# wx-ys/pynbody-extras

Hardware: AMD Instinct MI355X
Metric: particle-pairs/sec (direct-sum gravity, force+potential) (higher is better)
Workload: dtype f64; 1 GPU; 1000000-particle Plummer sphere, direct-sum force+potential (Newtonian), 1000000 targets/GPU x 1000000 sources; n_particles=1000000, seed=1002, parallelism=targets sharded x1, device=gfx950 device (gfx950:sramecc+:xnack-, 256 CUs)

## Files before the change

### pynbody-extras_amd/csrc/direct.hip

```cpp
#include <cstdlib>
#include <cstring>

#include "pbx_common.h"

namespace pbx {

static constexpr double kR2Tiny = 2.2250738585072014e-308;
static constexpr int kBlock = 256;

__device__ __forceinline__ double rsqrt_nr(double x) {
  double y = __builtin_amdgcn_rsq(x);
  double e = __builtin_fma(-x * y, y, 1.0);
  return __builtin_fma(0.5 * y, e, y);
}

__device__ __forceinline__ double w2_inner(double u) {
  double u2 = u * u;
  if (u < 0.5) {
    double u4 = u2 * u2;
    double u5 = u4 * u;
    return (16.0 / 3.0) * u2 - (48.0 / 5.0) * u4 + (32.0 / 5.0) * u5 - 14.0 / 5.0;
  }
  double inv_u = 1.0 / u;
  double u3 = u2 * u;
  double u4 = u2 * u2;
  double u5 = u4 * u;
  return (1.0 / 15.0) * inv_u + (32.0 / 3.0) * u2 - 16.0 * u3 + (48.0 / 5.0) * u4 -
         (32.0 / 15.0) * u5 - 16.0 / 5.0;
}

__device__ __forceinline__ double w2p_inner(double u) {
  double u2 = u * u;
  double u3 = u2 * u;
  double u4 = u2 * u2;
  if (u < 0.5) return (32.0 / 3.0) * u - (192.0 / 5.0) * u3 + 32.0 * u4;
  return -(1.0 / 15.0) * (1.0 / u2) + (64.0 / 3.0) * u - 48.0 * u2 + (192.0 / 5.0) * u3 -
         (32.0 / 3.0) * u4;
}

template <int KERN, int WANT>
__device__ __forceinline__ void pair(double dx, double dy, double dz, double m, double h,
                                     double &ph, double &ax, double &ay, double &az) {
  double s2 = __builtin_fma(dx, dx, __builtin_fma(dy, dy, __builtin_fma(dz, dz, kR2Tiny)));
  const double s = (KERN == 0) ? __builtin_fma(h, h, s2) : s2;
  const double y0 = __builtin_amdgcn_rsq(s);
  const double w = y0 * __builtin_fma(-s, y0 * y0, 3.0);
  double mw = m * w;
  double g8 = mw * (w * w);
  if (KERN == 1) {
    double r = s2 * (0.5 * w);
    if (!(h <= 0.0) && !(r >= h)) {
      double hinv = 1.0 / h;
      double u = r * hinv;
      mw = -2.0 * m * (w2_inner(u) * hinv);
      g8 = 8.0 * m * (w2p_inner(u) * (hinv * hinv) / r);
    }
  }
  if (WANT & PBX_WANT_POT) ph += mw;
  if (WANT & PBX_WANT_ACC) {
    ax = __builtin_fma(g8, dx, ax);
    ay = __builtin_fma(g8, dy, ay);
    az = __builtin_fma(g8, dz, az);
  }
}

template <int KERN, int WANT, bool CHECK, int T>
__device__ __forceinline__ void sweep(const double4 *__restrict__ src,
                                      const double *__restrict__ src_h, bool has_h,
                                      int64_t j0, int64_t j1, const double (&xi)[T],
                                      const double (&yi)[T], const double (&zi)[T],
                                      const double (&hi)[T], const int64_t (&me)[T],
                                      double (&ph)[T], double (&ax)[T], double (&ay)[T],
                                      double (&az)[T]) {
#pragma unroll 4
  for (int64_t j = j0; j < j1; ++j) {
    const double4 s = src[j];
    double hj = 0.0;
    if (KERN >= 0) hj = has_h ? src_h[j] : 0.0;
#pragma unroll
    for (int k = 0; k < T; ++k) {
      double dx = s.x - xi[k];
      double dy = s.y - yi[k];
      double dz = s.z - zi[k];
      double m = s.w;
      double h = 0.0;
      if (KERN >= 0) h = __builtin_fmax(hi[k], hj);
      if (CHECK) {
        bool self = (j == me[k]);
        m = self ? 0.0 : m;
        dx = self ? 1.0 : dx;
        if (KERN >= 0) h = self ? 0.0 : h;
      }
      pair<KERN, WANT>(dx, dy, dz, m, h, ph[k], ax[k], ay[k], az[k]);
    }
  }
}

template <int KERN, int WANT, bool SELF, int T>
__global__ void __launch_bounds__(kBlock)
    direct_kernel(const double4 *__restrict__ src, const double *__restrict__ src_h,
                  int has_h, int64_t n_src, int64_t chunk, const double *__restrict__ tgt,
                  const double *__restrict__ tgt_h, int64_t n_tgt, int64_t self_offset,
                  double *__restrict__ pot_out, double *__restrict__ acc_out,
                  int64_t out_split_stride) {
  const int64_t tbase = (int64_t)blockIdx.x * (kBlock * T);
  const int64_t js = (int64_t)blockIdx.y * chunk;
  const int64_t je = (js + chunk < n_src) ? js + chunk : n_src;

  double xi[T], yi[T], zi[T], hi[T], ph[T], ax[T], ay[T], az[T];
  int64_t me[T];
#pragma unroll
  for (int k = 0; k < T; ++k) {
    int64_t t = tbase + k * kBlock + threadIdx.x;
    int64_t tc = t < n_tgt ? t : n_tgt - 1;
    xi[k] = tgt[3 * tc + 0];
    yi[k] = tgt[3 * tc + 1];
    zi[k] = tgt[3 * tc + 2];
    hi[k] = (SELF && KERN >= 0 && has_h) ? tgt_h[tc] : 0.0;
    me[k] = SELF ? self_offset + t : -1;
    ph[k] = ax[k] = ay[k] = az[k] = 0.0;
  }

  const bool hh = has_h != 0;
  if (SELF) {
    int64_t d0 = self_offset + tbase;
    int64_t d1 = d0 + kBlock * T;
    d0 = d0 < js ? js : (d0 > je ? je : d0);
    d1 = d1 < js ? js : (d1 > je ? je : d1);
    sweep<KERN, WANT, false, T>(src, src_h, hh, js, d0, xi, yi, zi, hi, me, ph, ax, ay, az);
    sweep<KERN, WANT, true, T>(src, src_h, hh, d0, d1, xi, yi, zi, hi, me, ph, ax, ay, az);
    sweep<KERN, WANT, false, T>(src, src_h, hh, d1, je, xi, yi, zi, hi, me, ph, ax, ay, az);
  } else {
    sweep<KERN, WANT, false, T>(src, src_h, hh, js, je, xi, yi, zi, hi, me, ph, ax, ay, az);
  }

  const int64_t soff = (int64_t)blockIdx.y * out_split_stride;
#pragma unroll
  for (int k = 0; k < T; ++k) {
    int64_t t = tbase + k * kBlock + threadIdx.x;
    if (t < n_tgt) {
      if (WANT & PBX_WANT_POT) pot_out[soff + t] = -0.5 * ph[k];
      if (WANT & PBX_WANT_ACC) {
        double *a = acc_out + 3 * (soff + t);
        a[0] = 0.125 * ax[k];
        a[1] = 0.125 * ay[k];
        a[2] = 0.125 * az[k];
      }
    }
  }
}

template <int WANT>
__global__ void __launch_bounds__(kBlock)
    reduce_splits(const double *__restrict__ pot_part, const double *__restrict__ acc_part,
                  int nsplit, int64_t n_tgt, double *__restrict__ pot,
                  double *__restrict__ acc) {
  int64_t t = (int64_t)blockIdx.x * kBlock + threadIdx.x;
  if (t >= n_tgt) return;
  if (WANT & PBX_WANT_POT) {
    double s = 0.0;
    for (int k = 0; k < nsplit; ++k) s += pot_part[(int64_t)k * n_tgt + t];
    pot[t] = s;
  }
  if (WANT & PBX_WANT_ACC) {
    double sx = 0.0, sy = 0.0, sz = 0.0;
    for (int k = 0; k < nsplit; ++k) {
      const double *a = acc_part + 3 * ((int64_t)k * n_tgt + t);
      sx += a[0];
      sy += a[1];
      sz += a[2];
    }
    acc[3 * t + 0] = sx;
    acc[3 * t + 1] = sy;
    acc[3 * t + 2] = sz;
  }
}

__global__ void __launch_bounds__(kBlock)
    pack_sources_kernel(const double *__restrict__ pos, const double *__restrict__ mass,
                        int64_t n, double4 *__restrict__ rec) {
  int64_t i = (int64_t)blockIdx.x * kBlock + threadIdx.x;
  if (i >= n) return;
  rec[i] = make_double4(pos[3 * i + 0], pos[3 * i + 1], pos[3 * i + 2],
                        mass ? mass[i] : 1.0);
}

constexpr int kTargetsPerLane = 4;

template <int KERN, int WANT, bool SELF>
static void launch_variant(hipStream_t st, dim3 grid, const double4 *src, const double *src_h,
                           int has_h, int64_t n_src, int64_t chunk, const double *tgt,
                           const double *tgt_h, int64_t n_tgt, int64_t self_offset,
                           double *pot, double *acc, int64_t stride) {
  hipLaunchKernelGGL((direct_kernel<KERN, WANT, SELF, kTargetsPerLane>), grid, dim3(kBlock), 0,
                     st, src, src_h, has_h, n_src, chunk, tgt, tgt_h, n_tgt, self_offset, pot, acc,
                     stride);
}

template <int KERN, int WANT>
static void launch_self(bool self, hipStream_t st, dim3 grid, const double4 *src,
                        const double *src_h, int has_h, int64_t n_src, int64_t chunk,
                        const double *tgt, const double *tgt_h, int64_t n_tgt,
                        int64_t self_offset, double *pot, double *acc, int64_t stride) {
  if (self)
    launch_variant<KERN, WANT, true>(st, grid, src, src_h, has_h, n_src, chunk, tgt, tgt_h,
                                     n_tgt, self_offset, pot, acc, stride);
  else
    launch_variant<KERN, WANT, false>(st, grid, src, src_h, has_h, n_src, chunk, tgt, tgt_h,
                                      n_tgt, self_offset, pot, acc, stride);
}

template <int KERN>
static void launch_want(int want, bool self, hipStream_t st, dim3 grid, const double4 *src,
                        const double *src_h, int has_h, int64_t n_src, int64_t chunk,
                        const double *tgt, const double *tgt_h, int64_t n_tgt,
                        int64_t self_offset, double *pot, double *acc, int64_t stride) {
  switch (want) {
    case 1:
      launch_self<KERN, 1>(self, st, grid, src, src_h, has_h, n_src, chunk, tgt, tgt_h, n_tgt,
                           self_offset, pot, acc, stride);
      break;
    case 2:
      launch_self<KERN, 2>(self, st, grid, src, src_h, has_h, n_src, chunk, tgt, tgt_h, n_tgt,
                           self_offset, pot, acc, stride);
      break;
    default:
      launch_self<KERN, 3>(self, st, grid, src, src_h, has_h, n_src, chunk, tgt, tgt_h, n_tgt,
                           self_offset, pot, acc, stride);
      break;
  }
}

int64_t sym_padded(int64_t n);
int64_t sym_unit_count(int64_t n);
void sym_accumulate(Device &d, double4 *rec, int64_t n, int64_t u0, int64_t u1, int want,
                    double *acc4, DevBuf &unit_buf);
void sym_finish(Device &d, const double *acc4, int64_t lo, int64_t hi, int want, double *pot,
                double *acc);

static constexpr int64_t kSymMinN = 8192;

void direct_device(Device &d, const double *src, const double *src_h, int64_t n_src,
                   const double *tgt, const double *tgt_h, int64_t n_tgt, int64_t self_offset,
                   int kernel, int want, double *pot, double *acc) {
  if (n_tgt <= 0) return;
  hipStream_t st = d.stream;
  if (kernel == PBX_KERNEL_NONE && self_offset == 0 && n_tgt == n_src && n_src >= kSymMinN) {
    const int64_t npad = sym_padded(n_src);
    double4 *rec = (double4 *)d.slot(kSlotSymRec).ensure(sizeof(double4) * npad);
    double *acc4 = (double *)d.slot(kSlotSymAcc).ensure(sizeof(double) * 4 * npad);
    PBX_HIP(hipMemcpyAsync(rec, src, sizeof(double4) * n_src, hipMemcpyDeviceToDevice, st));
    PBX_HIP(hipMemsetAsync(acc4, 0, sizeof(double) * 4 * npad, st));
    sym_accumulate(d, rec, n_src, 0, sym_unit_count(n_src), want, acc4, d.slot(kSlotSymUnits));
    sym_finish(d, acc4, 0, n_src, want, pot, acc);
    return;
  }
  if (n_src <= 0) {
    if (want & PBX_WANT_POT) PBX_HIP(hipMemsetAsync(pot, 0, sizeof(double) * n_tgt, st));
    if (want & PBX_WANT_ACC) PBX_HIP(hipMemsetAsync(acc, 0, sizeof(double) * 3 * n_tgt, st));
    return;
  }
  const int64_t per_block = (int64_t)kBlock * kTargetsPerLane;
  const int64_t bx = (n_tgt + per_block - 1) / per_block;
  int64_t nsplit = (2048 + bx - 1) / bx;
  int64_t max_split = (n_src + 4095) / 4096;
  if (nsplit > max_split) nsplit = max_split;
  if (nsplit > 64) nsplit = 64;
  if (nsplit < 1) nsplit = 1;
  const int64_t chunk = (n_src + nsplit - 1) / nsplit;
  nsplit = (n_src + chunk - 1) / chunk;
  if (bx > 0x7fffffff) fail(PBX_ERR_VALUE, "too many targets (%lld)", (long long)n_tgt);
  dim3 grid((unsigned)bx, (unsigned)nsplit);
  const bool self = self_offset >= 0;
  const int has_h = src_h != nullptr;

  double *pot_k = pot, *acc_k = acc;
  int64_t stride = 0;
  if (nsplit > 1) {
    size_t per = 0;
    if (want & PBX_WANT_POT) per += 1;
    if (want & PBX_WANT_ACC) per += 3;
    double *part = (double *)d.slot(kSlotPart).ensure(sizeof(double) * per * nsplit * n_tgt);
    pot_k = (want & PBX_WANT_POT) ? part : nullptr;
    acc_k = (want & PBX_WANT_ACC) ? part + ((want & PBX_WANT_POT) ? nsplit * n_tgt : 0)
                                  : nullptr;
    stride = n_tgt;
  }
  const double4 *src4 = (const double4 *)src;
  switch (kernel) {
    case PBX_KERNEL_NONE:
      launch_want<-1>(want, self, st, grid, src4, src_h, has_h, n_src, chunk, tgt, tgt_h,
                      n_tgt, self_offset, pot_k, acc_k, stride);
      break;
    case PBX_KERNEL_PLUMMER:
      launch_want<0>(want, self, st, grid, src4, src_h, has_h, n_src, chunk, tgt, tgt_h,
                     n_tgt, self_offset, pot_k, acc_k, stride);
      break;
    case PBX_KERNEL_SPLINE:
      launch_want<1>(want, self, st, grid, src4, src_h, has_h, n_src, chunk, tgt, tgt_h,
                     n_tgt, self_offset, pot_k, acc_k, stride);
      break;
    default:
      fail(PBX_ERR_VALUE, "kernel must be 0 (Plummer) or 1 (CubicSplineW2)");
  }
  PBX_HIP(hipGetLastError());
  if (nsplit > 1) {
    dim3 rg(ceil_div(n_tgt, kBlock));
    switch (want) {
      case 1:
        hipLaunchKernelGGL(reduce_splits<1>, rg, dim3(kBlock), 0, st, pot_k, acc_k,
                           (int)nsplit, n_tgt, pot, acc);
        break;
      case 2:
        hipLaunchKernelGGL(reduce_splits<2>, rg, dim3(kBlock), 0, st, pot_k, acc_k,
                           (int)nsplit, n_tgt, pot, acc);
        break;
      default:
        hipLaunchKernelGGL(reduce_splits<3>, rg, dim3(kBlock), 0, st, pot_k, acc_k,
                           (int)nsplit, n_tgt, pot, acc);
        break;
    }
    PBX_HIP(hipGetLastError());
  }
}

void pack_sources_device(Device &d, const double *pos, const double *mass, int64_t n,
                         double *rec) {
  if (n <= 0) return;
  hipLaunchKernelGGL(pack_sources_kernel, dim3(ceil_div(n, kBlock)), dim3(kBlock), 0, d.stream,
                     pos, mass, n, (double4 *)rec);
  PBX_HIP(hipGetLastError());
}

static void check_kernel(int kernel, const double *soft) {
  if (kernel != PBX_KERNEL_NONE && kernel != PBX_KERNEL_PLUMMER && kernel != PBX_KERNEL_SPLINE)
    fail(PBX_ERR_VALUE, "kernel must be 0 (Plummer) or 1 (CubicSplineW2)");
  if (kernel == PBX_KERNEL_NONE && soft != nullptr)
    fail(PBX_ERR_VALUE,
         "softenings require an explicit kernel; pass kernel=0/1 (or omit softenings)");
}

static void direct_host(const double *h_pos, int64_t n, const double *h_tgt, int64_t m,
                        const double *h_mass, const double *h_soft, int kernel, int want,
                        double *h_out) {
  if (n < 0 || m < 0) fail(PBX_ERR_VALUE, "negative particle count");
  check_kernel(kernel, h_soft);
  const bool self = (h_tgt == nullptr);
  const int64_t n_tgt = self ? n : m;
  if (n_tgt == 0) return;
  Device &d = current_device();
  std::lock_guard<std::mutex> lk(d.mu);
  hipStream_t st = d.stream;
  size_t out_elems = (want == PBX_WANT_POT ? 1 : 3) * (size_t)n_tgt;
  if (n == 0) {
    std::memset(h_out, 0, sizeof(double) * out_elems);
    return;
  }
  ScopedTimer total("pbx.direct.total");
  double *d_pos = (double *)d.slot(kSlotPos).ensure(sizeof(double) * 3 * n);
  double *d_mass = h_mass ? (double *)d.slot(kSlotMass).ensure(sizeof(double) * n) : nullptr;
  double *d_src = (double *)d.slot(kSlotSrc).ensure(sizeof(double) * 4 * n);
  const bool use_h = h_soft != nullptr && kernel != PBX_KERNEL_NONE;
  double *d_src_h = use_h ? (double *)d.slot(kSlotSrcH).ensure(sizeof(double) * n) : nullptr;
  double *d_tgt = self ? d_pos : (double *)d.slot(kSlotTgt).ensure(sizeof(double) * 3 * m);
  double *d_out = (double *)d.slot(want == PBX_WANT_POT ? kSlotPot : kSlotAcc)
                      .ensure(sizeof(double) * out_elems);
  {
    ScopedTimer t("pbx.direct.h2d");
    PBX_HIP(hipMemcpyAsync(d_pos, h_pos, sizeof(double) * 3 * n, hipMemcpyHostToDevice, st));
    if (h_mass)
      PBX_HIP(hipMemcpyAsync(d_mass, h_mass, sizeof(double) * n, hipMemcpyHostToDevice, st));
    if (use_h)
      PBX_HIP(hipMemcpyAsync(d_src_h, h_soft, sizeof(double) * n, hipMemcpyHostToDevice, st));
    if (!self)
      PBX_HIP(hipMemcpyAsync(d_tgt, h_tgt, sizeof(double) * 3 * m, hipMemcpyHostToDevice, st));
    if (timing_enabled()) PBX_HIP(hipStreamSynchronize(st));
  }
  {
    ScopedTimer t("pbx.direct.compute");
    pack_sources_device(d, d_pos, d_mass, n, d_src);
    direct_device(d, d_src, d_src_h, n, d_tgt, self ? d_src_h : nullptr, n_tgt,
                  self ? 0 : -1, kernel, want, want == PBX_WANT_POT ? d_out : nullptr,
                  want == PBX_WANT_ACC ? d_out : nullptr);
    if (timing_enabled()) PBX_HIP(hipStreamSynchronize(st));
  }
  {
    ScopedTimer t("pbx.direct.d2h");
    PBX_HIP(hipMemcpyAsync(h_out, d_out, sizeof(double) * out_elems, hipMemcpyDeviceToHost, st));
    PBX_HIP(hipStreamSynchronize(st));
  }
}

}

using namespace pbx;

extern "C" {

int pbx_direct_accelerations(const double *h_pos, int64_t n, const double *h_masses,
                             const double *h_softenings, int kernel, double *h_acc) {
  return guard([&] {
    direct_host(h_pos, n, nullptr, 0, h_masses, h_softenings, kernel, PBX_WANT_ACC, h_acc);
  });
}

int pbx_direct_potentials(const double *h_pos, int64_t n, const double *h_masses,
                          const double *h_softenings, int kernel, double *h_pot) {
  return guard([&] {
    direct_host(h_pos, n, nullptr, 0, h_masses, h_softenings, kernel, PBX_WANT_POT, h_pot);
  });
}

int pbx_direct_accelerations_at_points(const double *h_pos, int64_t n, const double *h_targets,
                                       int64_t m, const double *h_masses,
                                       const double *h_softenings, int kernel, double *h_acc) {
  return guard([&] {
    if (m > 0 && !h_targets) fail(PBX_ERR_VALUE, "targets must be (N,3) float64 array");
    direct_host(h_pos, n, h_targets ? h_targets : h_pos, m, h_masses, h_softenings, kernel,
                PBX_WANT_ACC, h_acc);
  });
}

int pbx_direct_potentials_at_points(const double *h_pos, int64_t n, const double *h_targets,
                                    int64_t m, const double *h_masses,
                                    const double *h_softenings, int kernel, double *h_pot) {
  return guard([&] {
    if (m > 0 && !h_targets) fail(PBX_ERR_VALUE, "targets must be (N,3) float64 array");
    direct_host(h_pos, n, h_targets ? h_targets : h_pos, m, h_masses, h_softenings, kernel,
                PBX_WANT_POT, h_pot);
  });
}

int pbx_pack_sources(const double *d_pos, const double *d_mass, int64_t n, double *d_records) {
  return guard([&] {
    if (n < 0) fail(PBX_ERR_VALUE, "negative particle count");
    Device &d = current_device();
    pack_sources_device(d, d_pos, d_mass, n, d_records);
  });
}

int pbx_direct_dev(const double *d_src, const double *d_src_h, int64_t n_src,
                   const double *d_tgt, const double *d_tgt_h, int64_t n_tgt,
                   int64_t self_offset, int kernel, int want, double *d_pot, double *d_acc) {
  return guard([&] {
    if (n_src < 0 || n_tgt < 0) fail(PBX_ERR_VALUE, "negative particle count");
    if (want < 1 || want > 3) fail(PBX_ERR_VALUE, "want must be 1 (pot), 2 (acc) or 3");
    if ((want & PBX_WANT_POT) && !d_pot && n_tgt) fail(PBX_ERR_VALUE, "d_pot is NULL");
    if ((want & PBX_WANT_ACC) && !d_acc && n_tgt) fail(PBX_ERR_VALUE, "d_acc is NULL");
    if (kernel != PBX_KERNEL_NONE && kernel != PBX_KERNEL_PLUMMER && kernel != PBX_KERNEL_SPLINE)
      fail(PBX_ERR_VALUE, "kernel must be 0 (Plummer) or 1 (CubicSplineW2)");
    if (self_offset >= 0 && self_offset + n_tgt > n_src)
      fail(PBX_ERR_VALUE, "self_offset + n_tgt exceeds n_src");
    if (self_offset >= 0 && kernel != PBX_KERNEL_NONE && d_src_h && !d_tgt_h)
      fail(PBX_ERR_VALUE, "all-particles softened form needs d_tgt_h");
    Device &d = current_device();
    std::lock_guard<std::mutex> lk(d.mu);
    direct_device(d, d_src, kernel == PBX_KERNEL_NONE ? nullptr : d_src_h, n_src, d_tgt,
                  d_tgt_h, n_tgt, self_offset, kernel, want, d_pot, d_acc);
  });
}

}
```

### pynbody-extras_amd/csrc/direct_sym.hip

```cpp
#include <algorithm>
#include <type_traits>
#include <vector>

#include "pbx_common.h"

namespace pbx {
namespace sym {

static constexpr double kR2Tiny = 2.2250738585072014e-308;
constexpr int kWaves = 4;
#ifndef PBX_SYM_KT
#define PBX_SYM_KT 12
#endif
#ifndef PBX_SYM_KS
#define PBX_SYM_KS 2
#endif
constexpr int kT = PBX_SYM_KT;
constexpr int kS = PBX_SYM_KS;
constexpr int kBlk = 64 * kT;
constexpr int kChunk = 64 * kS;
constexpr int kJPerI = kBlk / kChunk;
constexpr int kSuper = kWaves * kBlk;
static_assert(kJPerI * kChunk == kBlk, "an I-block is a whole number of J-chunks");

struct Unit {
  int32_t sb;
  int32_t j0;
  int32_t j1;
  int32_t pad;
};

__device__ __forceinline__ double rot(double v, int addr) {
  const uint64_t b = __builtin_bit_cast(uint64_t, v);
  const int lo = __builtin_amdgcn_ds_bpermute(addr, (int)(uint32_t)b);
  const int hi = __builtin_amdgcn_ds_bpermute(addr, (int)(uint32_t)(b >> 32));
  return __builtin_bit_cast(double, ((uint64_t)(uint32_t)hi << 32) | (uint64_t)(uint32_t)lo);
}

__device__ __forceinline__ double rot_dpp(double v) {
  const uint64_t b = __builtin_bit_cast(uint64_t, v);
  const int l0 = (int)(uint32_t)b, h0 = (int)(uint32_t)(b >> 32);
  const int lo = __builtin_amdgcn_update_dpp(l0, l0, 0x134, 0xF, 0xF, false);
  const int hi = __builtin_amdgcn_update_dpp(h0, h0, 0x134, 0xF, 0xF, false);
  return __builtin_bit_cast(double, ((uint64_t)(uint32_t)hi << 32) | (uint64_t)(uint32_t)lo);
}
#ifndef PBX_SYM_DPP_MASK
#define PBX_SYM_DPP_MASK 0xFF
#endif

template <int WANT, bool SYMM, bool RAW, bool UNI, int DOFF = 0>
__device__ __forceinline__ void chunk(const double4 *__restrict__ rec, int64_t jbase, int lane,
                                      const double (&tx)[kT], const double (&ty)[kT],
                                      const double (&tz)[kT], const double (&tm)[kT],
                                      double (&tp)[kT], double (&ta)[kT], double (&tb)[kT],
                                      double (&tc)[kT], double (&sp)[kS], double (&sa)[kS],
                                      double (&sb)[kS], double (&sc)[kS]) {
  double sx[kS], sy[kS], sz[kS], sm[kS];
#pragma unroll
  for (int k = 0; k < kS; ++k) {
    const double4 r = rec[jbase + k * 64 + lane];
    sx[k] = r.x;
    sy[k] = r.y;
    sz[k] = r.z;
    sm[k] = UNI ? 0.0 : r.w;
    sp[k] = sa[k] = sb[k] = sc[k] = 0.0;
  }
  const int addr = ((lane + 1) & 63) << 2;
  for (int r = 0; r < 64; ++r) {
#pragma unroll
    for (int ks = 0; ks < kS; ++ks) {
#pragma unroll
      for (int kt = 0; kt < kT; ++kt) {
        double dx = sx[ks] - tx[kt], dy = sy[ks] - ty[kt], dz = sz[ks] - tz[kt];
        double ms = sm[ks];
        bool self = false;
        if (!SYMM && kt == DOFF * kS + ks) {
          self = (r == 0);
          ms = self ? 0.0 : ms;
          dx = self ? 1.0 : dx;
        }
        const double s2 =
            __builtin_fma(dx, dx, __builtin_fma(dy, dy, __builtin_fma(dz, dz, kR2Tiny)));
        const double y0 = __builtin_amdgcn_rsq(s2);
        double w = RAW ? y0 : y0 * __builtin_fma(-s2, y0 * y0, 3.0);
        if (UNI && !SYMM && kt == DOFF * kS + ks) w = self ? 0.0 : w;
        const double q = w * (w * w);
        if (WANT & PBX_WANT_POT) tp[kt] = UNI ? tp[kt] + w : __builtin_fma(ms, w, tp[kt]);
        if (WANT & PBX_WANT_ACC) {
          const double g = UNI ? q : ms * q;
          ta[kt] = __builtin_fma(g, dx, ta[kt]);
          tb[kt] = __builtin_fma(g, dy, tb[kt]);
          tc[kt] = __builtin_fma(g, dz, tc[kt]);
        }
        if (SYMM) {
          if (WANT & PBX_WANT_POT) sp[ks] = UNI ? sp[ks] + w : __builtin_fma(tm[kt], w, sp[ks]);
          if (WANT & PBX_WANT_ACC) {
            const double g = UNI ? q : tm[kt] * q;
            sa[ks] = __builtin_fma(-g, dx, sa[ks]);
            sb[ks] = __builtin_fma(-g, dy, sb[ks]);
            sc[ks] = __builtin_fma(-g, dz, sc[ks]);
          }
        }
      }
      auto rt = [&](double x, int bit) {
        return ((PBX_SYM_DPP_MASK >> bit) & 1) ? rot_dpp(x) : rot(x, addr);
      };
      sx[ks] = rt(sx[ks], 0);
      sy[ks] = rt(sy[ks], 1);
      sz[ks] = rt(sz[ks], 2);
      if (!UNI) sm[ks] = rt(sm[ks], 3);
      if (SYMM) {
        if (WANT & PBX_WANT_POT) sp[ks] = rt(sp[ks], 4);
        if (WANT & PBX_WANT_ACC) {
          sa[ks] = rt(sa[ks], 5);
          sb[ks] = rt(sb[ks], 6);
          sc[ks] = rt(sc[ks], 7);
        }
      }
    }
  }
}

template <int WANT, bool RAW, bool UNI, int D>
__device__ __forceinline__ void own_chunk(int d, const double4 *__restrict__ rec, int64_t jbase,
                                          int lane, const double (&tx)[kT], const double (&ty)[kT],
                                          const double (&tz)[kT], const double (&tm)[kT],
                                          double (&tp)[kT], double (&ta)[kT], double (&tb)[kT],
                                          double (&tc)[kT], double (&sp)[kS], double (&sa)[kS],
                                          double (&sb)[kS], double (&sc)[kS]) {
  if (d == D)
    chunk<WANT, false, RAW, UNI, D>(rec, jbase, lane, tx, ty, tz, tm, tp, ta, tb, tc, sp, sa, sb, sc);
  else if constexpr (D + 1 < kJPerI)
    own_chunk<WANT, RAW, UNI, D + 1>(d, rec, jbase, lane, tx, ty, tz, tm, tp, ta, tb, tc, sp, sa, sb,
                                     sc);
}

template <int WANT, bool RAW, bool UNI>
__global__ void __launch_bounds__(kWaves * 64)
    sym_kernel(const double4 *__restrict__ rec, const Unit *__restrict__ units,
               double *__restrict__ acc4, double m) {
  __shared__ double jl[kWaves][4][kChunk];
  const Unit u = units[blockIdx.x];
  const int w = threadIdx.x >> 6, lane = threadIdx.x & 63;
  const int64_t iblk = (int64_t)u.sb * kWaves + w;
  double tx[kT], ty[kT], tz[kT], tm[kT], tp[kT], ta[kT], tb[kT], tc[kT];
#pragma unroll
  for (int k = 0; k < kT; ++k) {
    const double4 r = rec[iblk * kBlk + k * 64 + lane];
    tx[k] = r.x;
    ty[k] = r.y;
    tz[k] = r.z;
    tm[k] = UNI ? 0.0 : r.w;
    tp[k] = ta[k] = tb[k] = tc[k] = 0.0;
  }
  const int64_t jdiag = iblk * kJPerI;
  for (int32_t j = u.j0; j < u.j1; ++j) {
    double sp[kS], sa[kS], sb[kS], sc[kS];
#pragma unroll
    for (int k = 0; k < kS; ++k) sp[k] = sa[k] = sb[k] = sc[k] = 0.0;
    if (j >= jdiag + kJPerI)
      chunk<WANT, true, RAW, UNI>(rec, (int64_t)j * kChunk, lane, tx, ty, tz, tm, tp, ta, tb, tc, sp,
                                  sa, sb, sc);
    else if (j >= jdiag)
      own_chunk<WANT, RAW, UNI, 0>((int)(j - jdiag), rec, (int64_t)j * kChunk, lane, tx, ty, tz, tm,
                                   tp, ta, tb, tc, sp, sa, sb, sc);
#pragma unroll
    for (int k = 0; k < kS; ++k) {
      jl[w][0][k * 64 + lane] = sp[k];
      jl[w][1][k * 64 + lane] = sa[k];
      jl[w][2][k * 64 + lane] = sb[k];
      jl[w][3][k * 64 + lane] = sc[k];
    }
    __syncthreads();
    if ((int64_t)j >= ((int64_t)u.sb * kWaves + 1) * kJPerI) {
      double *dst = acc4 + (int64_t)j * kChunk * 4;
      static_assert(kWaves * 64 * kS == kChunk * 4, "kS (source, quantity) words per thread");
#pragma unroll
      for (int i = 0; i < kS; ++i) {
        const int idx = threadIdx.x + i * kWaves * 64;
        const int s = idx >> 2, q = idx & 3;
        double v = jl[0][q][s] + jl[1][q][s] + jl[2][q][s] + jl[3][q][s];
        if (UNI) v *= m;
        if (v != 0.0) atomicAdd(dst + idx, v);
      }
    }
    __syncthreads();
  }
#pragma unroll
  for (int k = 0; k < kT; ++k) {
    double *dst = acc4 + (iblk * kBlk + k * 64 + lane) * 4;
    if (WANT & PBX_WANT_POT) atomicAdd(dst + 0, UNI ? m * tp[k] : tp[k]);
    if (WANT & PBX_WANT_ACC) {
      atomicAdd(dst + 1, UNI ? m * ta[k] : ta[k]);
      atomicAdd(dst + 2, UNI ? m * tb[k] : tb[k]);
      atomicAdd(dst + 3, UNI ? m * tc[k] : tc[k]);
    }
  }
}

__global__ void pad_records(double4 *__restrict__ rec, int64_t n, int64_t npad) {
  int64_t i = n + (int64_t)blockIdx.x * 256 + threadIdx.x;
  if (i >= npad) return;
  const double far = 1e100 * (double)(i - n + 1);
  rec[i] = make_double4(far, -far, 2.0 * far, 0.0);
}

struct MassProbe {
  double m;
  uint32_t differs;
  uint32_t pad;
};
__global__ void mass_probe(const double4 *__restrict__ rec, int64_t n,
                           MassProbe *__restrict__ out) {
  const int64_t i = (int64_t)blockIdx.x * 256 + threadIdx.x;
  const double m0 = rec[0].w;
  if (i == 0) out->m = m0;
  if (i < n && __builtin_bit_cast(uint64_t, rec[i].w) != __builtin_bit_cast(uint64_t, m0))
    out->differs = 1u;
}

__global__ void finish_kernel(const double *__restrict__ acc4, int64_t lo, int64_t hi, int want,
                              int raw, double *__restrict__ pot, double *__restrict__ acc) {
  int64_t t = (int64_t)blockIdx.x * 256 + threadIdx.x;
  if (lo + t >= hi) return;
  const double *a = acc4 + (lo + t) * 4;
  const double kp = raw ? -1.0 : -0.5, ka = raw ? 1.0 : 0.125;
  if (want & PBX_WANT_POT) pot[t] = kp * a[0];
  if (want & PBX_WANT_ACC) {
    acc[3 * t + 0] = ka * a[1];
    acc[3 * t + 1] = ka * a[2];
    acc[3 * t + 2] = ka * a[3];
  }
}

}

int64_t sym_padded(int64_t n) {
  return (n + sym::kSuper - 1) / sym::kSuper * sym::kSuper;
}

#ifndef PBX_SYM_CHUNKS_PER_UNIT
#define PBX_SYM_CHUNKS_PER_UNIT 32
#endif
static std::vector<sym::Unit> sym_units(int64_t npad) {
  constexpr int kChunksPerUnit = PBX_SYM_CHUNKS_PER_UNIT;
  const int32_t nch = (int32_t)(npad / sym::kChunk);
  const int32_t nsb = (int32_t)(npad / sym::kSuper);
  std::vector<sym::Unit> u;
  for (int32_t sb = 0; sb < nsb; ++sb)
    for (int32_t j = sb * sym::kWaves * sym::kJPerI; j < nch; j += kChunksPerUnit)
      u.push_back({sb, j, std::min(nch, j + kChunksPerUnit), 0});
  return u;
}

int64_t sym_unit_count(int64_t n) { return (int64_t)sym_units(sym_padded(n)).size(); }

static sym::MassProbe sym_probe_mass(Device &d, const double4 *rec, int64_t n) {
  hipStream_t st = d.stream;
  sym::MassProbe *dp = (sym::MassProbe *)d.slot(kSlotSymProbe).ensure(sizeof(sym::MassProbe));
  sym::MassProbe h{};
  const bool timed = timing_enabled();
  hipEvent_t e0 = nullptr, e1 = nullptr;
  if (timed) {
    PBX_HIP(hipEventCreate(&e0));
    PBX_HIP(hipEventCreate(&e1));
    PBX_HIP(hipEventRecord(e0, st));
  }
  PBX_HIP(hipMemsetAsync(dp, 0, sizeof(sym::MassProbe), st));
  hipLaunchKernelGGL(sym::mass_probe, dim3(ceil_div(n, 256)), dim3(256), 0, st, rec, n, dp);
  PBX_HIP(hipGetLastError());
  PBX_HIP(hipMemcpyAsync(&h, dp, sizeof(sym::MassProbe), hipMemcpyDeviceToHost, st));
  if (timed) PBX_HIP(hipEventRecord(e1, st));
  PBX_HIP(hipStreamSynchronize(st));
  if (timed) {
    float ms = 0.f;
    PBX_HIP(hipEventElapsedTime(&ms, e0, e1));
    std::fprintf(stderr, "[pynbodyext-timing] direct_sym mass probe (n=%lld): %.4f ms\n",
                 (long long)n, (double)ms);
    (void)hipEventDestroy(e0);
    (void)hipEventDestroy(e1);
  }
  return h;
}


void sym_accumulate(Device &d, double4 *rec, int64_t n, int64_t u0, int64_t u1, int want,
                    double *acc4, DevBuf &unit_buf) {
  const int64_t npad = sym_padded(n);
  hipStream_t st = d.stream;
  if (npad > n)
    hipLaunchKernelGGL(sym::pad_records, dim3(ceil_div(npad - n, 256)), dim3(256), 0, st, rec, n,
                       npad);
  std::vector<sym::Unit> all = sym_units(npad);
  u0 = std::max<int64_t>(0, u0);
  u1 = std::min<int64_t>((int64_t)all.size(), u1);
  if (u1 <= u0) return;
  std::vector<sym::Unit> mine(all.begin() + u0, all.begin() + u1);
  std::stable_sort(mine.begin(), mine.end(), [](const sym::Unit &a, const sym::Unit &b) {
    return (a.j1 - a.j0) > (b.j1 - b.j0);
  });
  sym::Unit *du = (sym::Unit *)unit_buf.ensure(sizeof(sym::Unit) * mine.size());
  PBX_HIP(hipMemcpyAsync(du, mine.data(), sizeof(sym::Unit) * mine.size(), hipMemcpyHostToDevice,
                         st));
  const sym::MassProbe probe = sym_probe_mass(d, rec, n);
  const bool uni = probe.differs == 0;
  const double m = probe.m;
  const dim3 grid((unsigned)mine.size()), block(sym::kWaves * 64);
  auto launch = [&](auto raw, auto uniform) {
    constexpr bool R = decltype(raw)::value, U = decltype(uniform)::value;
    if (want == PBX_WANT_POT)
      hipLaunchKernelGGL((sym::sym_kernel<PBX_WANT_POT, R, U>), grid, block, 0, st, rec, du, acc4,
                         m);
    else if (want == PBX_WANT_ACC)
      hipLaunchKernelGGL((sym::sym_kernel<PBX_WANT_ACC, R, U>), grid, block, 0, st, rec, du, acc4,
                         m);
    else
      hipLaunchKernelGGL((sym::sym_kernel<PBX_WANT_POT | PBX_WANT_ACC, R, U>), grid, block, 0, st,
                         rec, du, acc4, m);
  };
  auto launch_raw = [&](auto raw) {
    if (uni)
      launch(raw, std::true_type{});
    else
      launch(raw, std::false_type{});
  };
  if (precise_mode())
    launch_raw(std::false_type{});
  else
    launch_raw(std::true_type{});
  ++(uni ? d.sym_uniform_launches : d.sym_general_launches);
  PBX_HIP(hipGetLastError());
  PBX_HIP(hipStreamSynchronize(st));
}

void sym_finish(Device &d, const double *acc4, int64_t lo, int64_t hi, int want, double *pot,
                double *acc) {
  if (hi <= lo) return;
  hipLaunchKernelGGL(sym::finish_kernel, dim3(ceil_div(hi - lo, 256)), dim3(256), 0, d.stream,
                     acc4, lo, hi, want, precise_mode() ? 0 : 1, pot, acc);
  PBX_HIP(hipGetLastError());
}

}

using namespace pbx;

extern "C" {

int pbx_direct_sym_plan(int64_t n, int64_t *npad, int64_t *n_units, int64_t *h_weights) {
  return guard([&] {
    if (n < 0) fail(PBX_ERR_VALUE, "negative particle count");
    const int64_t np = sym_padded(n);
    std::vector<sym::Unit> u = sym_units(np);
    if (npad) *npad = np;
    if (n_units) *n_units = (int64_t)u.size();
    if (h_weights)
      for (size_t i = 0; i < u.size(); ++i) h_weights[i] = u[i].j1 - u[i].j0;
  });
}

int pbx_direct_sym_accumulate(const double *d_src, int64_t n, int64_t u0, int64_t u1, int want,
                              double *d_acc4) {
  return guard([&] {
    if (n < 0) fail(PBX_ERR_VALUE, "negative particle count");
    if (want < 1 || want > 3) fail(PBX_ERR_VALUE, "want must be 1 (pot), 2 (acc) or 3");
    if (n == 0) return;
    Device &d = current_device();
    std::lock_guard<std::mutex> lk(d.mu);
    const int64_t npad = sym_padded(n);
    double4 *rec = (double4 *)d.slot(kSlotSymRec).ensure(sizeof(double4) * npad);
    PBX_HIP(hipMemcpyAsync(rec, d_src, sizeof(double4) * n, hipMemcpyDeviceToDevice, d.stream));
    sym_accumulate(d, rec, n, u0, u1, want, d_acc4, d.slot(kSlotSymUnits));
  });
}

int pbx_direct_sym_path_stats(int64_t *uniform_launches, int64_t *general_launches) {
  return guard([&] {
    Device &d = current_device();
    std::lock_guard<std::mutex> lk(d.mu);
    if (uniform_launches) *uniform_launches = d.sym_uniform_launches;
    if (general_launches) *general_launches = d.sym_general_launches;
  });
}

int pbx_direct_sym_finish(const double *d_acc4, int64_t lo, int64_t hi, int want, double *d_pot,
                          double *d_acc) {
  return guard([&] {
    if (lo < 0 || hi < lo) fail(PBX_ERR_VALUE, "bad particle range");
    Device &d = current_device();
    std::lock_guard<std::mutex> lk(d.mu);
    sym_finish(d, d_acc4, lo, hi, want, d_pot, d_acc);
    PBX_HIP(hipStreamSynchronize(d.stream));
  });
}

}
```

### pynbody-extras_amd/csrc/pbx_common.h

```cpp
#pragma once

#include <hip/hip_runtime.h>

#include <chrono>
#include <condition_variable>
#include <cstdarg>
#include <cstdint>
#include <cstdio>
#include <mutex>
#include <string>
#include <thread>
#include <vector>

#include "../../include/pbx.h"

namespace pbx {

void set_error(const char *fmt, ...);

struct Error {
  int code;
  std::string msg;
};

[[noreturn]] void fail(int code, const char *fmt, ...);

#define PBX_HIP(call)                                                        \
  do {                                                                       \
    hipError_t _e = (call);                                                  \
    if (_e != hipSuccess)                                                    \
      ::pbx::fail(PBX_ERR_RUNTIME, "%s failed: %s (%s:%d)", #call,           \
                  hipGetErrorString(_e), __FILE__, __LINE__);                \
  } while (0)

template <class F> int guard(F &&f) {
  try {
    f();
    return PBX_OK;
  } catch (const Error &e) {
    set_error("%s", e.msg.c_str());
    return e.code;
  } catch (const std::bad_alloc &) {
    set_error("host allocation failed");
    return PBX_ERR_RUNTIME;
  } catch (...) {
    set_error("unknown internal error");
    return PBX_ERR_RUNTIME;
  }
}

struct DevBuf {
  void *ptr = nullptr;
  size_t bytes = 0;
  void *ensure(size_t need);
  ~DevBuf();
};

void *dev_alloc(size_t need, size_t *got, int *dev);
void dev_release(void *p, size_t bytes, int dev);

struct Device {
  int id = -1;
  hipStream_t stream = nullptr;
  std::mutex mu;
  std::vector<DevBuf *> slots;
  DevBuf &slot(int k);
  std::vector<void *> ring;
  std::vector<hipEvent_t> ring_ev;
  std::vector<bool> ring_used;
  int64_t sym_uniform_launches = 0, sym_general_launches = 0;
};

enum Slot {
  kSlotSrc = 0,
  kSlotSrcH,
  kSlotTgt,
  kSlotTgtH,
  kSlotPos,
  kSlotMass,
  kSlotPot,
  kSlotAcc,
  kSlotPart,
  kSlotProf0,
  kSlotProf1,
  kSlotProf2,
  kSlotProf3,
  kSlotProf4,
  kSlotProf5,
  kSlotProf6,
  kSlotProf7,
  kSlotComm,
  kSlotSymRec,
  kSlotSymAcc,
  kSlotSymUnits,
  kSlotSymProbe,
  kSlotPropPos,
  kSlotPropVel,
  kSlotPropMass,
  kSlotPropPart,
  kSlotCount
};

Device &current_device();

void h2d_staged(Device &d, void *dst, const void *src, size_t bytes, hipStream_t st);
void d2h_staged(Device &d, void *dst, const void *src, size_t bytes, hipStream_t st);
bool d2h_staged_widen(Device &d, int64_t *dst, const int32_t *src, int64_t n, hipStream_t st);

bool timing_enabled();

struct ScopedTimer {
  const char *label;
  std::chrono::steady_clock::time_point t0;
  bool on;
  explicit ScopedTimer(const char *l)
      : label(l), t0(std::chrono::steady_clock::now()), on(timing_enabled()) {}
  ~ScopedTimer() {
    if (on) {
      double ms = std::chrono::duration<double, std::milli>(
                      std::chrono::steady_clock::now() - t0)
                      .count();
      std::fprintf(stderr, "[pynbodyext-timing] %s: %.3f ms\n", label, ms);
    }
  }
};

struct CommRanks {
  int nranks, rank;
};
CommRanks comm_ranks(void *comm);
void comm_allreduce(void *comm, const void *send, void *recv, int64_t count, int dtype, int op,
                    hipStream_t st, std::unique_lock<std::mutex> &lk);

bool precise_mode();
void set_precise_mode(bool on);

inline unsigned int ceil_div(int64_t a, int64_t b) {
  return (unsigned int)((a + b - 1) / b);
}

constexpr unsigned kNumXcd = 8;
__device__ __forceinline__ unsigned xcd_swizzle(unsigned b, unsigned nblocks) {
  const unsigned q = nblocks / kNumXcd, r = nblocks % kNumXcd;
  const unsigned x = b % kNumXcd, k = b / kNumXcd;
  return (x < r ? x * (q + 1) : r * (q + 1) + (x - r) * q) + k;
}
__device__ __forceinline__ unsigned xcd_chunk_swizzle(unsigned b, unsigned chunk) {
  const unsigned x = b % kNumXcd, k = b / kNumXcd;
  return ((k / chunk) * kNumXcd + x) * chunk + k % chunk;
}

}
```

Before: 3539 billion pairs/s.

## Stage source records in per-wave LDS image and cache unit table across calls

Each wave now writes its source chunk into a doubled LDS image, so it can read the rotated source positions and masses with plain LDS loads instead of lane rotations. Only the symmetric partial sums still rotate, now always through DPP. The change also forces two waves per EU, partially unrolls the rotation loop, and narrows some index arithmetic to 32 bits. On the host, the sorted unit table is cached across calls and the trailing stream synchronize is dropped, which removes per-call host sorting, copying and blocking. The costs are extra LDS use and occupancy pressure, plus a cached table that has to stay consistent.

```diff
diff --git a/pynbody-extras_amd/csrc/direct.hip b/pynbody-extras_amd/csrc/direct.hip
--- a/pynbody-extras_amd/csrc/direct.hip
+++ b/pynbody-extras_amd/csrc/direct.hip
@@ -234,7 +234,7 @@
 int64_t sym_padded(int64_t n);
 int64_t sym_unit_count(int64_t n);
 void sym_accumulate(Device &d, double4 *rec, int64_t n, int64_t u0, int64_t u1, int want,
-                    double *acc4, DevBuf &unit_buf);
+                    double *acc4);
 void sym_finish(Device &d, const double *acc4, int64_t lo, int64_t hi, int want, double *pot,
                 double *acc);
 
@@ -251,7 +251,7 @@
     double *acc4 = (double *)d.slot(kSlotSymAcc).ensure(sizeof(double) * 4 * npad);
     PBX_HIP(hipMemcpyAsync(rec, src, sizeof(double4) * n_src, hipMemcpyDeviceToDevice, st));
     PBX_HIP(hipMemsetAsync(acc4, 0, sizeof(double) * 4 * npad, st));
-    sym_accumulate(d, rec, n_src, 0, sym_unit_count(n_src), want, acc4, d.slot(kSlotSymUnits));
+    sym_accumulate(d, rec, n_src, 0, sym_unit_count(n_src), want, acc4);
     sym_finish(d, acc4, 0, n_src, want, pot, acc);
     return;
   }
diff --git a/pynbody-extras_amd/csrc/direct_sym.hip b/pynbody-extras_amd/csrc/direct_sym.hip
--- a/pynbody-extras_amd/csrc/direct_sym.hip
+++ b/pynbody-extras_amd/csrc/direct_sym.hip
@@ -30,13 +30,6 @@
   int32_t pad;
 };
 
-__device__ __forceinline__ double rot(double v, int addr) {
-  const uint64_t b = __builtin_bit_cast(uint64_t, v);
-  const int lo = __builtin_amdgcn_ds_bpermute(addr, (int)(uint32_t)b);
-  const int hi = __builtin_amdgcn_ds_bpermute(addr, (int)(uint32_t)(b >> 32));
-  return __builtin_bit_cast(double, ((uint64_t)(uint32_t)hi << 32) | (uint64_t)(uint32_t)lo);
-}
-
 __device__ __forceinline__ double rot_dpp(double v) {
   const uint64_t b = __builtin_bit_cast(uint64_t, v);
   const int l0 = (int)(uint32_t)b, h0 = (int)(uint32_t)(b >> 32);
@@ -44,28 +37,62 @@
   const int hi = __builtin_amdgcn_update_dpp(h0, h0, 0x134, 0xF, 0xF, false);
   return __builtin_bit_cast(double, ((uint64_t)(uint32_t)hi << 32) | (uint64_t)(uint32_t)lo);
 }
-#ifndef PBX_SYM_DPP_MASK
-#define PBX_SYM_DPP_MASK 0xFF
-#endif
+
+#ifndef PBX_SYM_SRC_LDS
+#define PBX_SYM_SRC_LDS 1
+#endif
+constexpr bool kSrcLds = PBX_SYM_SRC_LDS != 0;
+
+constexpr int kImg = 2 * 64;
+struct WaveImage {
+  double2 src[kS][2][kImg];
+};
 
 template <int WANT, bool SYMM, bool RAW, bool UNI, int DOFF = 0>
 __device__ __forceinline__ void chunk(const double4 *__restrict__ rec, int64_t jbase, int lane,
-                                      const double (&tx)[kT], const double (&ty)[kT],
-                                      const double (&tz)[kT], const double (&tm)[kT],
-                                      double (&tp)[kT], double (&ta)[kT], double (&tb)[kT],
-                                      double (&tc)[kT], double (&sp)[kS], double (&sa)[kS],
-                                      double (&sb)[kS], double (&sc)[kS]) {
+                                      double2 *img, const double (&tx)[kT],
+                                      const double (&ty)[kT], const double (&tz)[kT],
+                                      const double (&tm)[kT], double (&tp)[kT], double (&ta)[kT],
+                                      double (&tb)[kT], double (&tc)[kT], double (&sp)[kS],
+                                      double (&sa)[kS], double (&sb)[kS], double (&sc)[kS]) {
   double sx[kS], sy[kS], sz[kS], sm[kS];
 #pragma unroll
   for (int k = 0; k < kS; ++k) {
-    const double4 r = rec[jbase + k * 64 + lane];
+    const double4 r = (rec + jbase + k * 64)[(unsigned)lane];
     sx[k] = r.x;
     sy[k] = r.y;
     sz[k] = r.z;
     sm[k] = UNI ? 0.0 : r.w;
     sp[k] = sa[k] = sb[k] = sc[k] = 0.0;
-  }
-  const int addr = ((lane + 1) & 63) << 2;
+    if (kSrcLds) {
+      double2 *s = img + k * 2 * kImg;
+      const double2 xy = make_double2(r.x, r.y), zm = make_double2(r.z, r.w);
+      s[0] = xy;
+      s[64] = xy;
+      s[kImg] = zm;
+      s[kImg + 64] = zm;
+    }
+  }
+  auto fetch = [&](int ks, int r) {
+    const double2 *s = img + ks * 2 * kImg + r;
+    const double2 xy = s[0];
+    sx[ks] = xy.x;
+    sy[ks] = xy.y;
+    if (UNI) {
+      sz[ks] = s[kImg].x;
+    } else {
+      const double2 zm = s[kImg];
+      sz[ks] = zm.x;
+      sm[ks] = zm.y;
+    }
+  };
+  if (kSrcLds) {
+    __builtin_amdgcn_fence(__ATOMIC_RELEASE, "wavefront");
+    __builtin_amdgcn_fence(__ATOMIC_ACQUIRE, "wavefront");
+#pragma unroll
+    for (int ks = 0; ks < kS; ++ks) fetch(ks, 0);
+  }
+#pragma unroll 4
   for (int r = 0; r < 64; ++r) {
 #pragma unroll
     for (int ks = 0; ks < kS; ++ks) {
@@ -102,19 +129,21 @@
           }
         }
       }
-      auto rt = [&](double x, int bit) {
-        return ((PBX_SYM_DPP_MASK >> bit) & 1) ? rot_dpp(x) : rot(x, addr);
-      };
-      sx[ks] = rt(sx[ks], 0);
-      sy[ks] = rt(sy[ks], 1);
-      sz[ks] = rt(sz[ks], 2);
-      if (!UNI) sm[ks] = rt(sm[ks], 3);
+      if (kSrcLds) {
+        __builtin_amdgcn_fence(__ATOMIC_ACQUIRE, "wavefront");
+        fetch(ks, r + 1);
+      } else {
+        sx[ks] = rot_dpp(sx[ks]);
+        sy[ks] = rot_dpp(sy[ks]);
+        sz[ks] = rot_dpp(sz[ks]);
+        if (!UNI) sm[ks] = rot_dpp(sm[ks]);
+      }
       if (SYMM) {
-        if (WANT & PBX_WANT_POT) sp[ks] = rt(sp[ks], 4);
+        if (WANT & PBX_WANT_POT) sp[ks] = rot_dpp(sp[ks]);
         if (WANT & PBX_WANT_ACC) {
-          sa[ks] = rt(sa[ks], 5);
-          sb[ks] = rt(sb[ks], 6);
-          sc[ks] = rt(sc[ks], 7);
+          sa[ks] = rot_dpp(sa[ks]);
+          sb[ks] = rot_dpp(sb[ks]);
+          sc[ks] = rot_dpp(sc[ks]);
         }
       }
     }
@@ -123,47 +152,57 @@
 
 template <int WANT, bool RAW, bool UNI, int D>
 __device__ __forceinline__ void own_chunk(int d, const double4 *__restrict__ rec, int64_t jbase,
-                                          int lane, const double (&tx)[kT], const double (&ty)[kT],
-                                          const double (&tz)[kT], const double (&tm)[kT],
-                                          double (&tp)[kT], double (&ta)[kT], double (&tb)[kT],
-                                          double (&tc)[kT], double (&sp)[kS], double (&sa)[kS],
-                                          double (&sb)[kS], double (&sc)[kS]) {
+                                          int lane, double2 *img, const double (&tx)[kT],
+                                          const double (&ty)[kT], const double (&tz)[kT],
+                                          const double (&tm)[kT], double (&tp)[kT],
+                                          double (&ta)[kT], double (&tb)[kT], double (&tc)[kT],
+                                          double (&sp)[kS], double (&sa)[kS], double (&sb)[kS],
+                                          double (&sc)[kS]) {
   if (d == D)
-    chunk<WANT, false, RAW, UNI, D>(rec, jbase, lane, tx, ty, tz, tm, tp, ta, tb, tc, sp, sa, sb, sc);
+    chunk<WANT, false, RAW, UNI, D>(rec, jbase, lane, img, tx, ty, tz, tm, tp, ta, tb, tc, sp, sa,
+                                    sb, sc);
   else if constexpr (D + 1 < kJPerI)
-    own_chunk<WANT, RAW, UNI, D + 1>(d, rec, jbase, lane, tx, ty, tz, tm, tp, ta, tb, tc, sp, sa, sb,
-                                     sc);
+    own_chunk<WANT, RAW, UNI, D + 1>(d, rec, jbase, lane, img, tx, ty, tz, tm, tp, ta, tb, tc, sp,
+                                     sa, sb, sc);
 }
 
 template <int WANT, bool RAW, bool UNI>
-__global__ void __launch_bounds__(kWaves * 64)
+__global__ void __launch_bounds__(kWaves * 64) __attribute__((amdgpu_waves_per_eu(2, 2)))
     sym_kernel(const double4 *__restrict__ rec, const Unit *__restrict__ units,
                double *__restrict__ acc4, double m) {
+#if PBX_SYM_SRC_LDS
+  __shared__ WaveImage image[kWaves];
+#endif
   __shared__ double jl[kWaves][4][kChunk];
   const Unit u = units[blockIdx.x];
   const int w = threadIdx.x >> 6, lane = threadIdx.x & 63;
-  const int64_t iblk = (int64_t)u.sb * kWaves + w;
+#if PBX_SYM_SRC_LDS
+  double2 *img = &image[w].src[0][0][lane];
+#else
+  double2 *img = nullptr;
+#endif
+  const int32_t iblk = u.sb * kWaves + w;
   double tx[kT], ty[kT], tz[kT], tm[kT], tp[kT], ta[kT], tb[kT], tc[kT];
 #pragma unroll
   for (int k = 0; k < kT; ++k) {
-    const double4 r = rec[iblk * kBlk + k * 64 + lane];
+    const double4 r = rec[(int64_t)iblk * kBlk + k * 64 + lane];
     tx[k] = r.x;
     ty[k] = r.y;
     tz[k] = r.z;
     tm[k] = UNI ? 0.0 : r.w;
     tp[k] = ta[k] = tb[k] = tc[k] = 0.0;
   }
-  const int64_t jdiag = iblk * kJPerI;
+  const int32_t jdiag = iblk * kJPerI;
   for (int32_t j = u.j0; j < u.j1; ++j) {
     double sp[kS], sa[kS], sb[kS], sc[kS];
 #pragma unroll
     for (int k = 0; k < kS; ++k) sp[k] = sa[k] = sb[k] = sc[k] = 0.0;
     if (j >= jdiag + kJPerI)
-      chunk<WANT, true, RAW, UNI>(rec, (int64_t)j * kChunk, lane, tx, ty, tz, tm, tp, ta, tb, tc, sp,
-                                  sa, sb, sc);
+      chunk<WANT, true, RAW, UNI>(rec, (int64_t)j * kChunk, lane, img, tx, ty, tz, tm, tp, ta, tb,
+                                  tc, sp, sa, sb, sc);
     else if (j >= jdiag)
-      own_chunk<WANT, RAW, UNI, 0>((int)(j - jdiag), rec, (int64_t)j * kChunk, lane, tx, ty, tz, tm,
-                                   tp, ta, tb, tc, sp, sa, sb, sc);
+      own_chunk<WANT, RAW, UNI, 0>((int)(j - jdiag), rec, (int64_t)j * kChunk, lane, img, tx, ty,
+                                   tz, tm, tp, ta, tb, tc, sp, sa, sb, sc);
 #pragma unroll
     for (int k = 0; k < kS; ++k) {
       jl[w][0][k * 64 + lane] = sp[k];
@@ -188,7 +227,7 @@
   }
 #pragma unroll
   for (int k = 0; k < kT; ++k) {
-    double *dst = acc4 + (iblk * kBlk + k * 64 + lane) * 4;
+    double *dst = acc4 + ((int64_t)jdiag * kChunk + k * 64) * 4 + lane * 4;
     if (WANT & PBX_WANT_POT) atomicAdd(dst + 0, UNI ? m * tp[k] : tp[k]);
     if (WANT & PBX_WANT_ACC) {
       atomicAdd(dst + 1, UNI ? m * ta[k] : ta[k]);
@@ -284,28 +323,47 @@
 }
 
 
+static const sym::Unit *sym_unit_table(Device &d, int64_t npad, int64_t u0, int64_t u1,
+                                       int64_t *count) {
+  DevBuf &buf = d.slot(kSlotSymUnits);
+  if (d.sym_table_npad == npad && d.sym_table_u0 == u0 && d.sym_table_u1 == u1 && buf.ptr) {
+    *count = d.sym_table_count;
+    return (const sym::Unit *)buf.ptr;
+  }
+  std::vector<sym::Unit> all = sym_units(npad);
+  const int64_t lo = std::max<int64_t>(0, u0), hi = std::min<int64_t>((int64_t)all.size(), u1);
+  *count = std::max<int64_t>(0, hi - lo);
+  if (*count == 0) return nullptr;
+  std::vector<sym::Unit> mine(all.begin() + lo, all.begin() + hi);
+  std::stable_sort(mine.begin(), mine.end(), [](const sym::Unit &a, const sym::Unit &b) {
+    return (a.j1 - a.j0) > (b.j1 - b.j0);
+  });
+  d.sym_table_npad = -1;
+  sym::Unit *du = (sym::Unit *)buf.ensure(sizeof(sym::Unit) * mine.size());
+  PBX_HIP(hipMemcpyAsync(du, mine.data(), sizeof(sym::Unit) * mine.size(), hipMemcpyHostToDevice,
+                         d.stream));
+  PBX_HIP(hipStreamSynchronize(d.stream));
+  d.sym_table_npad = npad;
+  d.sym_table_u0 = u0;
+  d.sym_table_u1 = u1;
+  d.sym_table_count = *count;
+  return du;
+}
+
 void sym_accumulate(Device &d, double4 *rec, int64_t n, int64_t u0, int64_t u1, int want,
-                    double *acc4, DevBuf &unit_buf) {
+                    double *acc4) {
   const int64_t npad = sym_padded(n);
   hipStream_t st = d.stream;
   if (npad > n)
     hipLaunchKernelGGL(sym::pad_records, dim3(ceil_div(npad - n, 256)), dim3(256), 0, st, rec, n,
                        npad);
-  std::vector<sym::Unit> all = sym_units(npad);
-  u0 = std::max<int64_t>(0, u0);
-  u1 = std::min<int64_t>((int64_t)all.size(), u1);
-  if (u1 <= u0) return;
-  std::vector<sym::Unit> mine(all.begin() + u0, all.begin() + u1);
-  std::stable_sort(mine.begin(), mine.end(), [](const sym::Unit &a, const sym::Unit &b) {
-    return (a.j1 - a.j0) > (b.j1 - b.j0);
-  });
-  sym::Unit *du = (sym::Unit *)unit_buf.ensure(sizeof(sym::Unit) * mine.size());
-  PBX_HIP(hipMemcpyAsync(du, mine.data(), sizeof(sym::Unit) * mine.size(), hipMemcpyHostToDevice,
-                         st));
+  int64_t count = 0;
+  const sym::Unit *du = sym_unit_table(d, npad, u0, u1, &count);
+  if (count == 0) return;
   const sym::MassProbe probe = sym_probe_mass(d, rec, n);
   const bool uni = probe.differs == 0;
   const double m = probe.m;
-  const dim3 grid((unsigned)mine.size()), block(sym::kWaves * 64);
+  const dim3 grid((unsigned)count), block(sym::kWaves * 64);
   auto launch = [&](auto raw, auto uniform) {
     constexpr bool R = decltype(raw)::value, U = decltype(uniform)::value;
     if (want == PBX_WANT_POT)
@@ -330,7 +388,6 @@
     launch_raw(std::true_type{});
   ++(uni ? d.sym_uniform_launches : d.sym_general_launches);
   PBX_HIP(hipGetLastError());
-  PBX_HIP(hipStreamSynchronize(st));
 }
 
 void sym_finish(Device &d, const double *acc4, int64_t lo, int64_t hi, int want, double *pot,
@@ -370,7 +427,7 @@
     const int64_t npad = sym_padded(n);
     double4 *rec = (double4 *)d.slot(kSlotSymRec).ensure(sizeof(double4) * npad);
     PBX_HIP(hipMemcpyAsync(rec, d_src, sizeof(double4) * n, hipMemcpyDeviceToDevice, d.stream));
-    sym_accumulate(d, rec, n, u0, u1, want, d_acc4, d.slot(kSlotSymUnits));
+    sym_accumulate(d, rec, n, u0, u1, want, d_acc4);
   });
 }
 
diff --git a/pynbody-extras_amd/csrc/pbx_common.h b/pynbody-extras_amd/csrc/pbx_common.h
--- a/pynbody-extras_amd/csrc/pbx_common.h
+++ b/pynbody-extras_amd/csrc/pbx_common.h
@@ -69,6 +69,7 @@
   std::vector<hipEvent_t> ring_ev;
   std::vector<bool> ring_used;
   int64_t sym_uniform_launches = 0, sym_general_launches = 0;
+  int64_t sym_table_npad = -1, sym_table_u0 = 0, sym_table_u1 = 0, sym_table_count = 0;
 };
 
 enum Slot {
```

Result: no change. 3567 billion pairs/s (median of 6 runs) (+0.8%).
